# PROBIC/mSWEEP

Hardware: AMD Instinct MI355X
Metric: EM iters/sec + reads×groups cells/sec, 10M reads × 5k groups (higher is better)
Workload: dtype f64

## Files before the change

include/msweep_core.h:

```cpp
#ifndef MSWEEP_CORE_H
#define MSWEEP_CORE_H

#include <stddef.h>
#include <stdint.h>

#ifdef __cplusplus
extern "C" {
#endif

typedef struct msw_core *msw_handle;

enum { MSW_ALGO_RCG = 0, MSW_ALGO_EM = 1 };
enum { MSW_PREC_DOUBLE = 0, MSW_PREC_FLOAT = 1 };

int msw_core_create(int device, msw_handle *out);
void msw_core_destroy(msw_handle h);
const char *msw_last_error(msw_handle h);
const char *msw_core_version(void);


int msw_core_set_dense_logl(msw_handle h, const double *L, size_t n_groups, size_t n_ecs,
                            size_t ld);

int msw_core_set_csr(msw_handle h, const uint64_t *rowptr, const uint32_t *grp,
// ... 15 lines not shown
  int32_t record_bytes;
  int32_t index_records;
  int32_t groups_in_lds;
  int32_t table_in_lds;
  int32_t passB_mode;
  uint32_t slot_entries;
  uint32_t slot_entries_in_lds;
  uint32_t n_slices, n_long_ecs;
  uint64_t rows;
  uint64_t rows_from_memory;
  uint32_t slices_by_lanes[7];
  uint32_t max_rows;
  int32_t bank_scheduled;
  int32_t passB_reg_cells;
  uint64_t rows_over_8;
} msw_layout_info;
int msw_core_layout_info(msw_handle h, msw_layout_info *out);
int msw_core_set_pack_schedule(msw_handle h, int enabled);

enum { MSW_OPT_CHECK_EVERY = 0, MSW_OPT_INIT_BOUND = 1, MSW_OPT_EM_PRIOR = 2, MSW_OPT_EM_STOP = 3 };
int msw_core_set_option(msw_handle h, int option, double value);
int msw_core_get_option(msw_handle h, int option, double *value);

int msw_core_solve(msw_handle h, const double *logc, const double *alpha0, double tol,
                   size_t max_iters, int algo, int prec, double *theta_out,
                   size_t *iters_out, double *bound_out);

int msw_core_prepare(msw_handle h, const double *logc, const double *alpha0);
int msw_core_run(msw_handle h, double tol, size_t max_iters, int algo, int prec,
                 double *theta_out, size_t *iters_out, double *bound_out);

int msw_core_gamma(msw_handle h, double *gamma_out, size_t ld);
// ... 127 lines not shown
```

msweep_amd/core.py:

```python
import ctypes as C
import os

import numpy as np

_HERE = os.path.dirname(os.path.abspath(__file__))
LIB_PATH = os.environ.get("MSWEEP_CORE_LIB") or os.path.join(_HERE, "libmsweep_core.so")

ALGO_RCG, ALGO_EM = 0, 1
PREC_DOUBLE, PREC_FLOAT = 0, 1
TEXT_PROBS, TEXT_LOGL, TEXT_BITSEQ = 0, 1, 2
OPT_CHECK_EVERY, OPT_INIT_BOUND, OPT_EM_PRIOR, OPT_EM_STOP = 0, 1, 2, 3
_OPTS = {"check_every": OPT_CHECK_EVERY, "init_bound": OPT_INIT_BOUND, "em_prior": OPT_EM_PRIOR, "em_stop": OPT_EM_STOP}

EXPORTS = [
    "msw_core_create", "msw_core_destroy", "msw_last_error", "msw_core_version",
    "msw_core_set_dense_logl", "msw_core_set_csr", "msw_core_build_likelihood",
    "msw_core_get_dense_logl", "msw_core_layout_hash", "msw_core_shape", "msw_alignment_read",
    "msw_alignment_shape", "msw_alignment_export", "msw_alignment_view", "msw_alignment_destroy", "msw_alignment_last_error",
    "msw_alignment_read_device", "msw_core_build_likelihood_aln", "msw_core_trim", "msw_alignment_on_device", "msw_core_solve", "msw_core_prepare", "msw_core_run",
    "msw_core_gamma",
    "msw_core_trace", "msw_core_set_trace_theta", "msw_core_bootstrap",
    "msw_core_resample_counts", "msw_core_set_profiling", "msw_core_last_timing",
    "msw_core_set_fixed_iters", "msw_core_hbm_stream_rates", "msw_comm_unique_id", "msw_comm_create_rccl", "msw_comm_create_local",
    "msw_comm_destroy", "msw_core_set_comm", "msw_comm_last_error", "msw_core_bootstrap_dist",
    "msw_comm_size", "msw_comm_rccl_count", "msw_comm_allgather", "msw_comm_allreduce", "msw_comm_create_shm", "msw_core_continue", "msw_core_gamma_block",
    "msw_core_last_bootstrap_timing", "msw_core_layout_info", "msw_core_guarded_visits", "msw_core_set_pack_schedule",
    "msw_core_set_option", "msw_core_get_option", "msw_core_bin_reads", "msw_core_bin_reads_aln",
    "msw_core_text_block", "msw_core_format_g6", "msw_core_last_text_timing",
    "msw_core_gzip_begin", "msw_core_text_block_gzip", "msw_core_gzip_append", "msw_core_gzip_end", "msw_core_last_gzip_timing",
    "msw_core_inflate_gzip", "msw_alignment_last_inflate",
]

INFLATE_REASONS = ("none", "forced", "header", "probe mismatch", "chunk status", "crc", "trailing bytes", "memory", "long span")


class MswError(RuntimeError):
    """Non-zero return from the C ABI (mirrors the std::runtime_error the C++ shim throws)."""


class InflateInfo(C.Structure):
    _fields_ = [("payload_bytes", C.c_uint64), ("text_bytes", C.c_uint64), ("chunk_bytes", C.c_uint32), ("n_chunks", C.c_uint32),
                ("n_starts", C.c_uint32), ("on_device", C.c_int32), ("fallback_reason", C.c_int32), ("n_members", C.c_uint32),
                ("kernel_ms", C.c_double),
                ("upload_ms", C.c_double), ("probe_ms", C.c_double), ("window_ms", C.c_double), ("chain_ms", C.c_double),
                ("write_ms", C.c_double), ("crc_ms", C.c_double)]
# ... 5 lines not shown


class Timing(C.Structure):
    _fields_ = [("solve_ms", C.c_double), ("passA_ms", C.c_double), ("passB_ms", C.c_double),
                ("passA_launches", C.c_uint64), ("passB_launches", C.c_uint64), ("iters", C.c_uint64),
                ("bytes_passA", C.c_uint64), ("bytes_passB", C.c_uint64), ("collective_ms", C.c_double),
                ("collectives", C.c_uint64), ("em_float_kernels", C.c_uint64)]


class LayoutInfo(C.Structure):
    _fields_ = [("record_bytes", C.c_int32), ("index_records", C.c_int32), ("groups_in_lds", C.c_int32),
                ("table_in_lds", C.c_int32), ("passB_mode", C.c_int32), ("slot_entries", C.c_uint32),
                ("slot_entries_in_lds", C.c_uint32), ("n_slices", C.c_uint32), ("n_long_ecs", C.c_uint32),
                ("rows", C.c_uint64), ("rows_from_memory", C.c_uint64), ("slices_by_lanes", C.c_uint32 * 7),
                ("max_rows", C.c_uint32), ("bank_scheduled", C.c_int32), ("passB_reg_cells", C.c_int32),
                ("rows_over_8", C.c_uint64)]


class BootstrapTiming(C.Structure):
    _fields_ = [("table_ms", C.c_double), ("solve_ms", C.c_double), ("gather_ms", C.c_double),
                ("replicates", C.c_uint64), ("iterations", C.c_uint64), ("table_reused", C.c_uint64)]


_lib = None


def source_hash():
    import hashlib
    csrc = os.path.join(_HERE, "csrc")
    h = hashlib.sha256()
    files = sorted(os.path.join(csrc, f) for f in os.listdir(csrc) if f.endswith((".hip", ".hpp", ".inc", ".h")))
# ... 66 lines not shown
    L.msw_comm_size.argtypes = [vp, C.POINTER(C.c_int), C.POINTER(C.c_int)]
    L.msw_comm_rccl_count.argtypes = [vp, C.POINTER(C.c_int)]
    L.msw_comm_allgather.argtypes = [vp, vp, sz, vp]
    L.msw_comm_allreduce.argtypes = [vp, vp, sz, vp, sz, C.c_int, C.POINTER(dp)]
    L.msw_comm_create_shm.argtypes = [C.c_char_p, C.c_int, C.c_int, C.c_int, C.POINTER(vp)]
    L.msw_core_set_profiling.argtypes = [vp, C.c_int]
    L.msw_core_set_fixed_iters.argtypes = [vp, C.c_int]
    L.msw_core_set_pack_schedule.argtypes = [vp, C.c_int]
    L.msw_core_set_option.argtypes = [vp, C.c_int, C.c_double]
    L.msw_core_get_option.argtypes = [vp, C.c_int, C.POINTER(C.c_double)]
    L.msw_core_hbm_stream_rates.argtypes = [vp, C.c_size_t, C.c_int, C.POINTER(C.c_double), C.POINTER(C.c_double)]
    L.msw_core_last_timing.argtypes = [vp, C.POINTER(Timing)]
    L.msw_core_last_bootstrap_timing.argtypes = [vp, C.POINTER(BootstrapTiming)]
    L.msw_core_guarded_visits.argtypes = [vp, C.POINTER(C.c_uint64)]
    L.msw_core_layout_info.argtypes = [vp, C.POINTER(LayoutInfo)]
    L.msw_comm_unique_id.argtypes = [vp]
    L.msw_comm_create_rccl.argtypes = [vp, C.c_int, C.c_int, C.c_int, C.POINTER(vp)]
    L.msw_comm_create_local.argtypes = [C.c_int, C.POINTER(vp)]
    L.msw_comm_destroy.argtypes = [vp]
    L.msw_comm_destroy.restype = None
    L.msw_core_set_comm.argtypes = [vp, vp]
    L.msw_comm_last_error.restype = C.c_char_p
    L.msw_alignment_read.argtypes = [C.POINTER(C.c_char_p), sz, sz, C.c_int, C.POINTER(vp)]
    L.msw_alignment_shape.argtypes = [vp, C.POINTER(sz), C.POINTER(sz), C.POINTER(sz), C.POINTER(sz)]
    L.msw_alignment_view.argtypes = [vp] + [C.POINTER(vp)] * 5
    L.msw_alignment_export.argtypes = [vp, vp, vp, vp, vp, vp]
    L.msw_alignment_destroy.argtypes = [vp]
    L.msw_core_trim.argtypes = [vp]
    L.msw_alignment_on_device.argtypes = [vp]
    L.msw_alignment_read_device.argtypes = [vp, C.POINTER(C.c_char_p), sz, sz, C.c_int, C.POINTER(vp)]
# ... 190 lines not shown
        self._check(self._L.msw_core_build_likelihood_aln(
            self._h, aln._h, _ptr(target_group), len(target_group), _ptr(group_sizes), G, q, e, zero_inflation,
            int(min_hits), C.byref(n_out), _ptr(mask), _ptr(logc)))
        return n_out.value, mask.astype(bool), logc

    def shape(self):
        g, e, n = C.c_size_t(), C.c_size_t(), C.c_size_t()
        self._check(self._L.msw_core_shape(self._h, C.byref(g), C.byref(e), C.byref(n)))
        return g.value, e.value, n.value

    def layout_info(self):
        t = LayoutInfo()
        self._check(self._L.msw_core_layout_info(self._h, C.byref(t)))
        return {k: (list(getattr(t, k)) if k == "slices_by_lanes" else getattr(t, k)) for k, _ in LayoutInfo._fields_}

    def layout_hash(self):
        out = C.c_uint64(0)
        self._check(self._L.msw_core_layout_hash(self._h, C.byref(out)))
        return int(out.value)

    def get_dense_logl(self):
        G, E, _ = self.shape()
        out = np.empty((G, E))
        self._check(self._L.msw_core_get_dense_logl(self._h, _ptr(out), E))
        return out

    def solve(self, logc, alpha0, tol=1e-6, max_iters=5000, algo=ALGO_RCG, prec=PREC_DOUBLE):
        G, E, _ = self.shape()
        logc = None if logc is None else _arr(logc, np.float64)
        alpha0 = _arr(alpha0, np.float64)
# ... 323 lines not shown
```

msweep_amd/csrc/common.hpp:

```cpp
#pragma once
#include <hip/hip_runtime.h>

#include <cstdint>
#include <cstdio>
#include <stdexcept>
#include <string>
#include <vector>

namespace msw {

constexpr int kWave = 64;
#ifndef MSW_PASS_THREADS_A
#define MSW_PASS_THREADS_A 1024
#endif
#ifndef MSW_PASS_THREADS_B
#define MSW_PASS_THREADS_B 768
#endif
#ifndef MSW_PASS_THREADS_B8
#define MSW_PASS_THREADS_B8 1024
#endif
constexpr int kPassThreads = MSW_PASS_THREADS_A;
constexpr int kPassThreadsB = MSW_PASS_THREADS_B;
constexpr int kPassThreadsB8 = MSW_PASS_THREADS_B8;
constexpr int kMaxTrace = 4096;
// ... 59 lines not shown
  int32_t em_prior = 0;
  int32_t em_stop = 0;
};

#ifdef MSW_STAMPS
__device__ unsigned long long g_stamps[64 * 40];
#define MSW_STAMP(it, K, p) (g_stamps[((it) & 63) * 40 + (K) * 8 + (p)] = __builtin_amdgcn_s_memrealtime())
#define MSW_STAMP_MAX(it, K, p) atomicMax(&g_stamps[((it) & 63) * 40 + (K) * 8 + (p)], (unsigned long long)__builtin_amdgcn_s_memrealtime())
#else
#define MSW_STAMP(it, K, p) ((void)0)
#define MSW_STAMP_MAX(it, K, p) ((void)0)
#endif

struct TabDev {
  double2 *A, *B;
};

struct Scalars {
  double a, os_a, step_a;
  double oldnorm, newnorm, beta;
  double bound, oldbound, bound_const;
  double tol, csum;
  double M, U, p0, kappa;
  double logzi;
  double fx_scale, fx_inv, fx_tscale, fx_tinv, xb, tmax, tmin;
  double tref;
  int32_t didreset, reset_pending, done, iter;
  int32_t have_eval, eval_pad;
  int32_t max_iters, fixed_iters, trace_theta, flavor;
  int32_t check_every, em_prior, em_stop, opt_pad;
  int32_t tab_ver, fx_shift;
// ... 4 lines not shown
```

msweep_amd/csrc/host_em.inc:

```
namespace {

void run_em(const Resident &L, Solver &s, size_t max_iters, int prec) {
  const int G = (int)L.G, n_lut = L.n_tab_inline();
  TraceDev tr{s.tr_bound.p, s.tr_newnorm.p, s.tr_beta.p, s.tr_theta.p, s.tr_reset.p};
  hipLaunchKernelGGL(k_em_init, dim3(1), dim3(1024), 0, s.stream, s.sc.p, G, n_lut, s.u.p, L.lut_area.p,
                     s.e.p, s.tabs());
  launch_tables(L, s);
  const bool f32 = prec == MSW_PREC_FLOAT && em_f32_layout_ok(L, s);
  struct Flag {
    Solver &s;
    ~Flag() { s.em_f32 = false; }
  } flag{s};
  s.em_f32 = f32;
  s.timing.em_float_kernels = f32 ? 1 : 0;
  if (f32) {
    s.e32.alloc((size_t)G + kSentinels);
    s.tab32.alloc(std::max<uint32_t>(L.n_area, 1));
    hipLaunchKernelGGL(k_em_f32_prep, dim3(1), dim3(1024), 0, s.stream, s.sc.p, G, (int)L.n_area, L.lut_area.p, s.e.p,
                       s.e32.p, s.tab32.p);
  }
  size_t enq = 0;
  while (enq < max_iters) {
    const size_t batch = std::min<size_t>(kIterBatch, max_iters - enq);
    for (size_t b = 0; b < batch; ++b) {
      launch_passB(L, s);
      hipLaunchKernelGGL(k_em_fin, dim3(1), dim3(1024), 0, s.stream, s.sc.p, G, n_lut, fin_npartS(L, s), fin_partS(L, s),
                         s.Nc.p, s.alpha0.p, s.u.p, s.logth.p, L.lut_area.p, s.e.p, s.tabs(), tr,
                         f32 ? s.e32.p : (float *)nullptr);
    }
    MSW_HIP(hipGetLastError());
    enq += batch;
    poll(s);
    if (s.sc_host->done) break;
  }
}

}
```

msweep_amd/csrc/host_likelihood.inc:

```
namespace {

void sell_from_device(msw_core *h, const uint32_t *d_rowptr, const uint32_t *d_grp, const uint32_t *d_idx,
                      const double *cell_val = nullptr);
bool compress_dense(msw_core *h, const double *Lm, size_t ld, const double *stage, size_t G, size_t E, bool force);

void reset_likelihood(msw_core *h) {
  Resident &L = h->lik;
  static_cast<LikShape &>(L) = LikShape{};
  h->solver.have_solution = false;
  h->solver.prepared = false;
  h->iperm.release();
  L.long_row = multilane() ? kLongRow : kLongRowOneLane;
  if (const char *lr = getenv("MSWEEP_LONG_ROW"))
    L.long_row = (uint32_t)std::min(std::max(atoi(lr), 16), (int)L.long_row);
}

constexpr uint8_t kRGroup[64] = {0, 0, 0, 0, 1, 1, 1, 1, 1, 1, 1, 1, 0, 0, 0, 0, 1, 1, 1, 1, 0, 0,
                                 0, 0, 0, 0, 0, 0, 1, 1, 1, 1, 2, 2, 2, 2, 3, 3, 3, 3, 3, 3, 3, 3,
                                 2, 2, 2, 2, 3, 3, 3, 3, 2, 2, 2, 2, 2, 2, 2, 2, 3, 3, 3, 3};

constexpr uint8_t kRPos[64] = {0, 1, 2,  3,  0,  1,  2,  3,  4,  5,  6,  7,  4,  5,  6,  7,  8,  9,  10, 11, 8, 9,
                               10, 11, 12, 13, 14, 15, 12, 13, 14, 15, 0,  1,  2,  3,  0,  1,  2,  3,  4,  5, 6, 7,
                               4,  5,  6,  7,  8,  9,  10, 11, 8,  9,  10, 11, 12, 13, 14, 15, 12, 13, 14, 15};

struct SlotPlan {
  std::vector<uint32_t> canon, hot_rank;
  uint32_t rep_base = 0, H = 0, sentinel_slot = 0;
};
SlotPlan plan_slot_area(msw_core *h, const std::vector<uint64_t> &freq) {
  Resident &L = h->lik;
  const uint32_t n_lut = L.n_lut;
  SlotPlan sp;
  std::vector<uint32_t> used;
  for (uint32_t i = 0; i < n_lut; ++i) if (freq[i]) used.push_back(i);
  if (used.empty()) used.push_back(0);
  std::vector<uint32_t> by_freq(used);
  std::stable_sort(by_freq.begin(), by_freq.end(), [&](uint32_t a, uint32_t b) { return freq[a] > freq[b]; });
  sp.canon.assign(std::max<uint32_t>(n_lut, 1), 0);
  sp.hot_rank.assign(std::max<uint32_t>(n_lut, 1), UINT32_MAX);
  sp.sentinel_slot = used[0];
  for (uint32_t tryH : {64u, 32u, 16u, 8u, 0u}) {
    if (tryH > used.size()) continue;
    sp.H = tryH;
    sp.rep_base = sp.H ? (uint32_t)((used.size() + 15) & ~(size_t)15) : (uint32_t)used.size();
    L.n_area = sp.rep_base + 8 * sp.H;
    choose_layout(L);
    if (L.tlds && L.glds && !L.wide()) break;
  }
  bool hybrid = false;
  if (!L.tlds) {
    sp.H = 0;
    sp.rep_base = (uint32_t)used.size();
    L.n_area = (uint32_t)used.size();
    choose_layout(L);
    hybrid = choose_hybrid_layout(L, h->no_hybrid);
    if (hybrid) sp.sentinel_slot = by_freq[0];
  }
  const std::vector<uint32_t> &order = hybrid ? by_freq : used;
  std::vector<uint32_t> area_slot(L.n_area, used[0]);
  for (uint32_t e = 0; e < order.size(); ++e) area_slot[e] = order[e], sp.canon[order[e]] = e;
  for (uint32_t j = 0; j < sp.H; ++j) {
    sp.hot_rank[by_freq[j]] = j;
    for (uint32_t c = 0; c < 8; ++c) area_slot[sp.rep_base + (j >> 1) * 16 + 2 * c + (j & 1)] = by_freq[j];
  }
  L.area_slot.upload(area_slot.data(), area_slot.size(), h->stream);
  L.lut_area.alloc(L.n_area);
  hipLaunchKernelGGL(k_gather_f64, dim3((L.n_area + 255) / 256), dim3(256), 0, h->stream, L.lut.p, L.area_slot.p,
                     L.n_area, L.lut_area.p);
  L.trange.alloc(2);
  hipLaunchKernelGGL(k_minmax, dim3(1), dim3(1024), 0, h->stream, L.lut_area.p, (uint64_t)L.n_area, 0, L.trange.p);
  MSW_HIP(hipGetLastError());
  MSW_HIP(hipStreamSynchronize(h->stream));
  return sp;
}

void finish_sell(msw_core *h) {
  Resident &L = h->lik;
  const uint32_t wg_for_slices = (L.nslices + (kPassThreads / 64) - 1) / (kPassThreads / 64);
  L.nblk = (int)std::max<uint32_t>(1, std::min<uint32_t>(std::max(wg_for_slices, L.n_long), (uint32_t)h->n_cu));
// ... 25 lines not shown
  const uint32_t E = L.E, G = L.G, n_lut = L.n_lut;
  const uint64_t nnz_all = rowptr[E];
  std::vector<uint64_t> freq(std::max<uint32_t>(n_lut, 1), 0);
  for (uint64_t k = 0; k < nnz_all; ++k) ++freq[cell_idx[k]];
  const SlotPlan sp = plan_slot_area(h, freq);
  const std::vector<uint32_t> &canon = sp.canon, &hot_rank = sp.hot_rank;
  const uint32_t rep_base = sp.rep_base;
  const std::vector<uint32_t> used = {sp.sentinel_slot};
  const bool wide = L.wide(), hybrid = L.hybrid();
  const int rw = wide ? 2 : 1;
  const RecDec dec = L.dec;
  const uint32_t n_hot = L.n_tab_lds;
  auto entry_of = [&](int lane, uint32_t idx) -> uint32_t {
    const uint32_t j = hot_rank[idx];
    if (lane < 0 || j == UINT32_MAX) return canon[idx];
    return rep_base + (j >> 1) * 16 + 2 * (kRPos[lane] >> 1) + (j & 1);
  };
  auto put_entry = [&](std::vector<uint32_t> &dst, size_t slot, uint32_t g, uint32_t entry, bool hot = false) {
    if (wide) {
      const uint2 r = Rec<kEncWide>::make(g, entry, dec);
      dst[2 * slot] = r.x;
      dst[2 * slot + 1] = r.y;
    } else if (hybrid) {
      dst[slot] = hot ? Rec<kEncIndex>::make_h(g, entry, dec) : Rec<kEncIndex>::make(g, entry, dec);
    } else {
      dst[slot] = Rec<kEncNarrow>::make(g, entry, dec);
    }
  };
  auto put = [&](std::vector<uint32_t> &dst, size_t slot, uint32_t g, uint32_t idx, int lane, bool hot = false) {
    put_entry(dst, slot, g, entry_of(lane, idx), hot);
  };
// ... 444 lines not shown
```

msweep_amd/csrc/host_pack.inc:

```
namespace {

uint64_t device_scan_u32(msw_core *h, uint32_t *d, uint64_t n, DevBuf<uint32_t> &tot, DevBuf<uint64_t> &gt);

void choose_value_layout(Resident &L) {
  L.enc = kEncValue;
  L.tlds = false;
  L.n_area = 0;
  L.n_tab_lds = 0;
  L.dec.shift = 0;
  L.dec.mask = 0;
  L.dec.bhi = L.dec.bhiA = 0;
  const char *force = getenv("MSWEEP_FORCE_LDS");
  const bool want_glds = !(force && strlen(force) == 2 && force[0] == '0');
  L.glds = want_glds && pass_lds_bytes(1, 0, L.G, true, false) <= kLdsMax && passB_mode(L, true, 0, false) >= 0;
  L.gmodeB = passB_mode(L, L.glds, 0, false);
  if (L.gmodeB < 0) throw Fail("internal: no LDS configuration fits");
  if (8ull * ((uint64_t)L.G + kSentinels) >= (1ull << 31)) throw Fail("likelihood too large: group offsets exceed the record field");
}

void sell_from_device(msw_core *h, const uint32_t *d_rowptr, const uint32_t *d_grp, const uint32_t *d_idx,
                      const double *cell_val ) {
  Resident &L = h->lik;
  const uint32_t E = L.E, n_lut = L.n_lut;
  const uint64_t nnz = L.nnz;
// ... 81 lines not shown
      sell_from_device(h, d_rowptr, d_grp, d_idx, cell_val);
    } catch (...) {
      h->no_hybrid = false;
      throw;
    }
    h->no_hybrid = false;
    return;
  }
  const size_t nslots = (size_t)n_rows * 64;
  if (L.hybrid()) L.slice_hot.alloc(std::max<uint32_t>(nslices, 1));
  L.rec.alloc(rec_words(L.enc, nslots + 64) + 2);
  L.rec_long.alloc(rec_words(L.enc, (size_t)n_long_cells + 64) + 2);
  MSW_HIP(hipMemsetAsync(L.rec.p + rec_words(L.enc, nslots), 0, (rec_words(L.enc, 64) + 2) * sizeof(uint32_t), st));
  MSW_HIP(hipMemsetAsync(L.rec_long.p, 0, (rec_words(L.enc, (size_t)n_long_cells + 64) + 2) * sizeof(uint32_t), st));
  tm.mark("  pack: geometry + alloc");
  const PackEnc pe{d_canon.p, d_hot.p, sp.rep_base, L.G, sp.sentinel_slot, L.dec, L.n_tab_lds, L.slice_hot.p,
                   cell_val, L.logzi};
  if (n_long) {
    auto k = L.enc == kEncValue ? k_pack_long<kEncValue>
                                 : (L.wide() ? k_pack_long<kEncWide> : (L.hybrid() ? k_pack_long<kEncIndex> : k_pack_long<kEncNarrow>));
    hipLaunchKernelGGL(k, dim3(std::min<uint32_t>(n_long, (uint32_t)h->n_cu * 32)), dim3(64), 0, st, d_rowptr, d_grp, d_idx,
                       L.perm.p, L.long_ptr.p, n_long, pe, L.rec_long.p);
  }
  if (nslices) {
    auto k = L.enc == kEncValue ? k_pack_slices<kEncValue>
                                 : (L.wide() ? k_pack_slices<kEncWide> : (L.hybrid() ? k_pack_slices<kEncIndex> : k_pack_slices<kEncNarrow>));
    hipLaunchKernelGGL(k, dim3(std::min<uint32_t>(nslices, (uint32_t)h->n_cu * 64)), dim3(64), 0, st, d_rowptr, d_grp,
                       d_idx, L.perm.p, L.slice_off.p, n_long, n_sell, nslices, L.cls, pe, h->pack_schedule ? 1 : 0, L.rec.p);
  }
  MSW_HIP(hipGetLastError());
  tm.mark("  pack: records");
// ... 39 lines not shown
```

msweep_amd/csrc/msweep_core.hip:

```cpp
#include "../../include/msweep_core.h"

#include <algorithm>
#include <array>
#include <cmath>
#include <chrono>
#include <cstring>
#include <limits>
#include <memory>
#include <string>
#include <thread>
#include <unordered_map>
#include <vector>

#include <zlib.h>

#include <rocprim/device/device_radix_sort.hpp>
#include <rocprim/device/device_scan.hpp>
#include <rocprim/iterator/counting_iterator.hpp>
#include <rocprim/iterator/transform_iterator.hpp>

#include "kernels.hpp"
#include "pack_kernels.hpp"
#include "compress_kernels.hpp"
#include "comm.hpp"
// ... 18 lines not shown
constexpr size_t kLdsMax = 160 * 1024;
constexpr int kIterBatch = 16;
}


struct LikShape {
  int flavor = -1;
  uint32_t G = 0, E = 0, n_lut = 0, nslices = 0, n_long = 0;
  uint64_t nnz = 0, nslots = 0;
  int enc = kEncNarrow;
  bool glds = true, tlds = true;
  int gmodeB = 1;
  RecDec dec = {};
  uint32_t n_area = 0;
  uint32_t n_tab_lds = 0;
  SliceClasses cls = {};
  bool packed_scheduled = false;
  uint32_t long_row = kLongRow;
  uint64_t rows_over8 = 0;
  bool passB_rc8 = false;
  double logzi = 0.0;
  int nblk = 0;
  int nblk_dense = 0;
  int nreg = 0;
  bool have_logc_res = false;
};

struct Resident : LikShape {
  DevBuf<uint32_t> rec, slice_off, long_ptr, rec_long, perm;
  DevBuf<uint8_t> slice_hot;
// ... 16 lines not shown

struct Solver {
  hipStream_t stream = nullptr;
  int n_cu = 256;
  msw_comm *const *commp;
  bool *collective;
  explicit Solver(msw_comm *const *c = nullptr, bool *coll = nullptr) : commp(c), collective(coll) {}
  msw_comm *comm() const { return commp ? *commp : nullptr; }
  SolveOpts opts;
  bool profiling = false, fixed_iters = false;
  size_t trace_theta = 0;

  DevBuf<double> cvec, logc_d, alpha0, u, os_u, step_u, w, e, N, Nc, Acc;
  DevBuf<uint8_t> c8, c8s;
  DevBuf<double2> ew, tabA, tabB;
  TabDev tabs() const { return TabDev{tabA.p, tabB.p}; }
  DevBuf<int> tab_built;
  DevBuf<double> partA, partS, partAcc, partC, partR, totS;
  size_t lds_attr[3][80] = {};
  DevBuf<double> commA, commB;
  DevBuf<uint32_t> guard_list, guard_bits;
  DevBuf<unsigned long long> guard_tail;
  DevBuf<int> guard_err;
  DevBuf<unsigned long long> guard_visits;
  DevBuf<Scalars> sc;
  Scalars *sc_host = nullptr;
  DevBuf<double> tr_bound, tr_newnorm, tr_beta, tr_theta;
  DevBuf<int32_t> tr_reset;
  bool have_solution = false;
  bool prepared = false;
  int last_algo = MSW_ALGO_RCG;
// ... 589 lines not shown
                       s.alpha0.p, s.Nc.p, s.N.p, s.w.p, s.ew.p, s.partR.p, s.totS.p);
    return;
  }
  hipLaunchKernelGGL(k_redfin, dim3((L.G + kRedfinGroups - 1) / kRedfinGroups), dim3(kRedfinThreads), 0, s.stream,
                     s.sc.p, (int)L.G, partials ? nb : 0, fxrows, fxrows ? s.guard_tail.p : nullptr, 1, nb,
                     s.partAcc.p, s.Acc.p, s.partS.p, s.e.p,
                     s.u.p, s.alpha0.p, s.Nc.p, s.N.p, s.w.p, s.ew.p, s.partR.p, s.totS.p);
}

const double *fin_partS(const Resident &L, Solver &s) { return s.comm() ? s.commB.p + 3 * (size_t)L.G : s.partS.p; }
int fin_npartS(const Resident &L, Solver &s) { return s.comm() ? 1 : L.npart_rows(); }

void launch_tables(const Resident &L, Solver &s) {
  if (L.flavor != 0 || L.n_area <= (uint32_t)kTabInline) return;
  const unsigned nb = std::min<unsigned>((L.n_area + 255) / 256, (unsigned)s.n_cu * 8);
  hipLaunchKernelGGL(k_tables, dim3(nb), dim3(256), 0, s.stream, s.sc.p, (int)L.n_area, L.lut_area.p, s.tabs(),
                     s.tab_built.p);
}

void launch_finstep(const Resident &L, Solver &s, int mode) {
  TraceDev tr{s.tr_bound.p, s.tr_newnorm.p, s.tr_beta.p, s.tr_theta.p, s.tr_reset.p};
  const double *pA = s.partA.p;
  int npA = L.flavor == 0 ? L.nblk : L.nblk_dense;
  if (s.comm()) {
    pA = s.commA.p;
    npA = 1;
  }
  hipLaunchKernelGGL(k_finstep, dim3(1), dim3(1024), 0, s.stream, s.sc.p, mode, (int)L.G, L.n_tab_inline(), npA, pA,
                     (int)((L.G + kRedfinGroups - 1) / kRedfinGroups), s.totS.p, s.partR.p, s.Nc.p, s.w.p, s.u.p,
                     s.os_u.p, s.step_u.p, L.lut_area.p, s.e.p, s.tabs(), tr);
  launch_tables(L, s);
}

void poll(Solver &s) {
  MSW_HIP(hipMemcpyAsync(s.sc_host, s.sc.p, sizeof(Scalars), hipMemcpyDeviceToHost, s.stream));
  MSW_HIP(hipStreamSynchronize(s.stream));
  if (s.comm()) s.comm()->check();
}

constexpr int kCvecBlocks = 512;
void prepare_inputs(const Resident &L, Solver &s, const double *logc_host, const uint32_t *counts_dev,
                    const double *alpha0_host) {
  if (L.flavor < 0) throw Fail("no likelihood resident: call msw_core_set_csr / set_dense_logl first");
  const uint32_t E = L.E, G = L.G;
  if (counts_dev) {
// ... 39 lines not shown
    cpart = s.commA.p;
    ncpart = 1;
  }
  hipLaunchKernelGGL(k_init_state, dim3(1), dim3(1024), 0, s.stream, s.sc.p, (int)G, ncpart,
                     cpart, s.alpha0.p, s.u.p, s.os_u.p, s.step_u.p, tol, (int)max_iters,
                     s.fixed_iters ? 1 : 0, (int)s.trace_theta, L.flavor, L.logzi, s.opts, s.tab_built.p,
                     L.trange.p);
  MSW_HIP(hipGetLastError());
}

void run_rcg(const Resident &L, Solver &s, size_t max_iters, size_t iters_start = 0) {
  const int G = (int)L.G, n_lut = L.n_tab_inline();
  if (iters_start > 0 && s.comm()) s.comm()->rendezvous();
  if (iters_start == 0) {
    hipLaunchKernelGGL(k_prepB, dim3(1), dim3(1024), 0, s.stream, s.sc.p, G, n_lut, s.u.p, L.lut_area.p,
                       s.e.p, s.tabs());
    launch_tables(L, s);
    launch_passB(L, s);
    s.timing.passB_launches--;
    if (s.profiling && s.evB_used) s.evB_used--;
  }
  const int nbA = L.flavor == 0 ? L.nblk : L.nblk_dense;
  size_t iters_done = iters_start;
  for (;;) {
    const size_t missing = std::max<size_t>(1, max_iters - std::min(max_iters, iters_done));
    const size_t batch = s.fixed_iters ? std::min<size_t>(256, missing) : std::min<size_t>(kIterBatch, missing);
    for (size_t b = 0; b < batch; ++b) {
      launch_passA(L, s);
      if (s.comm()) {
        std::pair<hipEvent_t, hipEvent_t> *evc = nullptr;
        if (s.profiling) {
// ... 311 lines not shown
    const Resident &L = h->lik;
    if (L.flavor != 0) throw Fail("msw_core_layout_info: no CSR-of-ECs likelihood resident");
    msw_layout_info li = {};
    li.record_bytes = L.enc == kEncValue ? 12 : (L.wide() ? 8 : 4);
    li.index_records = L.hybrid() ? 1 : 0;
    li.groups_in_lds = L.glds ? 1 : 0;
    li.table_in_lds = L.tlds ? 1 : 0;
    li.passB_mode = L.gmodeB;
    li.slot_entries = L.n_area;
    li.slot_entries_in_lds = L.n_tab_lds;
    li.n_slices = L.nslices;
    li.n_long_ecs = L.n_long;
    li.bank_scheduled = L.packed_scheduled ? 1 : 0;
    li.passB_reg_cells = L.passB_rc8 ? 8 : kRegCells;
    li.rows_over_8 = L.rows_over8;
    std::vector<uint32_t> off((size_t)L.nslices + 1);
    MSW_HIP(hipMemcpy(off.data(), L.slice_off.p, off.size() * sizeof(uint32_t), hipMemcpyDeviceToHost));
    li.rows = off[L.nslices];
    for (int c = 0; c < kSliceClasses; ++c) li.slices_by_lanes[c] = L.cls.s0[c + 1] - L.cls.s0[c];
    for (uint32_t s2 = 0; s2 < L.nslices; ++s2) li.max_rows = std::max(li.max_rows, off[s2 + 1] - off[s2]);
    if (L.hybrid()) {
      std::vector<uint8_t> hot(std::max<uint32_t>(L.nslices, 1));
      MSW_HIP(hipMemcpy(hot.data(), L.slice_hot.p, hot.size(), hipMemcpyDeviceToHost));
      for (uint32_t s2 = 0; s2 < L.nslices; ++s2) li.rows_from_memory += (off[s2 + 1] - off[s2]) - hot[s2];
    } else if (!L.tlds && L.enc != kEncValue) {
      li.rows_from_memory = li.rows;
    }
    *out = li;
  });
}

int msw_core_layout_hash(msw_handle h, uint64_t *hash_out) {
  return guarded(h, [&] {
    if (!hash_out) throw Fail("null out");
    *hash_out = layout_hash(h->lik);
  });
}

int msw_core_get_dense_logl(msw_handle h, double *L_out, size_t ld) {
  return guarded(h, [&] { materialise_impl(h, L_out, ld, false, 0, h->lik.E); });
}

int msw_core_gamma(msw_handle h, double *gamma_out, size_t ld) {
// ... 441 lines not shown
```

msweep_amd/csrc/pack_kernels.hpp:

```cpp
#pragma once
#include "common.hpp"
#include "sell.hpp"

namespace msw {

__device__ __constant__ uint8_t kRGroupDev[64] = {0, 0, 0, 0, 1, 1, 1, 1, 1, 1, 1, 1, 0, 0, 0, 0, 1, 1, 1, 1, 0, 0,
                                                  0, 0, 0, 0, 0, 0, 1, 1, 1, 1, 2, 2, 2, 2, 3, 3, 3, 3, 3, 3, 3, 3,
                                                  2, 2, 2, 2, 3, 3, 3, 3, 2, 2, 2, 2, 2, 2, 2, 2, 3, 3, 3, 3};
__device__ __constant__ uint8_t kRPosDev[64] = {0,  1,  2,  3,  0,  1,  2,  3,  4,  5,  6,  7,  4,  5,  6,  7,
                                                8,  9,  10, 11, 8,  9,  10, 11, 12, 13, 14, 15, 12, 13, 14, 15,
                                                0,  1,  2,  3,  0,  1,  2,  3,  4,  5,  6,  7,  4,  5,  6,  7,
                                                8,  9,  10, 11, 8,  9,  10, 11, 12, 13, 14, 15, 12, 13, 14, 15};

__host__ __device__ inline uint32_t cold_class(uint32_t n_cold) {
  return n_cold == 0 ? 0u : (n_cold <= 2 ? 1u : (n_cold <= (uint32_t)kColdRows ? 2u : 3u));
}
constexpr uint32_t kPackKeyBits = 13;
__global__ __launch_bounds__(256) void k_pack_keys(const uint32_t *rowptr, uint32_t E, uint32_t long_row, int multilane,
                                                  const uint32_t *idx, const uint32_t *canon, uint32_t n_hot,
                                                  uint32_t *key, uint32_t *val, uint32_t *counts) {
  uint32_t mine[1 + kSliceClasses] = {};
  for (uint32_t j = blockIdx.x * blockDim.x + threadIdx.x; j < E; j += gridDim.x * blockDim.x) {
    const uint32_t b = rowptr[j], len = rowptr[j + 1] - b;
    const bool lg = len > long_row;
// ... 54 lines not shown
    __syncthreads();
    for (uint32_t i = threadIdx.x; i < n_lut; i += blockDim.x)
      if (hist[i]) atomicAdd(&freq[i], (unsigned long long)hist[i]);
  }
}

__global__ __launch_bounds__(256) void k_gather_f64(const double *src, const uint32_t *at, uint32_t n, double *dst) {
  const uint32_t i = blockIdx.x * blockDim.x + threadIdx.x;
  if (i < n) dst[i] = src[at[i]];
}

struct PackEnc {
  const uint32_t *canon;
  const uint32_t *hot_rank;
  uint32_t rep_base, n_groups, sentinel_slot;
  RecDec dec;
  uint32_t n_hot;
  uint8_t *slice_hot;
  const double *cell_val;
  double tnull;
};
constexpr uint32_t kPackPad = UINT32_MAX;
__device__ __forceinline__ uint32_t pack_entry(const PackEnc &pe, int lane, uint32_t idx) {
  if (pe.cell_val) return idx;
  const uint32_t j = pe.hot_rank[idx];
  if (lane < 0 || j == UINT32_MAX) return pe.canon[idx];
  return pe.rep_base + (j >> 1) * 16 + 2 * (kRPosDev[lane] >> 1) + (j & 1);
}
template <int ENC>
__device__ __forceinline__ void pack_put(uint32_t *dst, size_t slot, const PackEnc &pe, uint32_t g, uint32_t entry,
                                         bool hot = false) {
  if constexpr (ENC == kEncValue) {
    Rec<ENC>::store(dst, slot, ValRec{8u * g, entry == kPackPad ? pe.tnull : pe.cell_val[entry]});
  } else {
    if (entry == kPackPad) entry = pe.canon[pe.sentinel_slot];
    if constexpr (ENC == kEncIndex) dst[slot] = hot ? Rec<ENC>::make_h(g, entry, pe.dec) : Rec<ENC>::make(g, entry, pe.dec);
    else reinterpret_cast<typename Rec<ENC>::T *>(dst)[slot] = Rec<ENC>::make(g, entry, pe.dec);
  }
}

constexpr uint32_t kLongResidues = 32;
__host__ __device__ inline uint32_t long_cell_pos(const uint32_t *b, uint32_t r, uint32_t j) {
// ... 196 lines not shown
```

msweep_amd/csrc/state_kernels.hpp:

```cpp
#pragma once
#include "device_util.hpp"

namespace msw {

struct TraceDev {
  double *bound, *newnorm, *beta, *theta;
  int32_t *didreset;
};

__device__ inline void prepB_block(Scalars *sc, double a, int G, int n_lut, const double *u,
                                   const double *lut, double *e, TabDev X, double *sh) {
  const int tid = threadIdx.x, nt = blockDim.x;
  double m = -INFINITY;
  for (int g = tid; g < G; g += nt) m = fmax(m, u[g]);
  const double M = block_max(m, sh);
  double su = 0.0;
  for (int g = tid; g < G; g += nt) {
    const double eg = flush_denormal(exp(u[g] - M));
    e[g] = eg;
    su += eg;
  }
  const double U = block_sum(su, sh);
  const double logzi = sc->logzi, oma = 1.0 - a;
  const double tref = tref_of(a, sc->tmax, sc->tmin);
  const double p0 = exp(a * (logzi - tref));
  const double xtop = 1.0;
  for (int i = tid; i < n_lut; i += nt) {
    const double T = lut[i], x = exp(a * (T - tref));
    X.A[i] = make_double2(x, oma * (T - logzi));
    X.B[i] = make_double2(x - p0, x * T - p0 * logzi);
  }
  if (tid == 0) {
    sc->M = M;
    sc->U = U;
    sc->p0 = p0;
    sc->tref = tref;
    sc->xb = fmax(xtop, p0);
    sc->fx_shift = fx_shift_of(fmax(xtop, p0), p0);
    sc->tab_ver = sc->tab_ver + 1;
  }
}

constexpr int kTabInline = 16384;
__global__ __launch_bounds__(256) void k_tables(const Scalars *sc, int n_tab, const double *lut, TabDev X,
                                               int *built) {
// ... 43 lines not shown
  __shared__ double sh[32];
  if (sc->done) return;
  if (sc->flavor != 0) return;
  const double a = sc->a;
  __syncthreads();
  prepB_block(sc, a, G, n_lut, u, lut, e, X, sh);
}

constexpr int kStepRegs = 6;
__global__ __launch_bounds__(1024) void k_finstep(Scalars *sc, int mode, int G, int n_lut, int n_partA,
                                                 const double *partA, int npartR, const double *totS,
                                                 const double *partR, const double *Nc, const double *w, double *u,
                                                 double *os_u, double *step_u, const double *lut, double *e, TabDev X,
                                                 TraceDev tr) {
  __shared__ double sh[16 * (kRedfinParts + 1)];
  const int tid = threadIdx.x, nt = blockDim.x;
  const bool inreg = G <= kStepRegs * nt;
  double q[kRedfinParts + 1] = {0.0, 0.0, 0.0, 0.0, 0.0, 0.0};
  for (int b = tid; b < npartR; b += nt)
    for (int i = 0; i < kRedfinParts; ++i) q[i] += partR[kRedfinParts * b + i];
  for (int i = tid; i < n_partA; i += nt) q[kRedfinParts] += partA[i];
  const double s_clogZ = totS[0], s_rH = totS[1];
  double wv[kStepRegs], sv[kStepRegs], uv[kStepRegs];
  if (inreg) {
#pragma unroll
    for (int k = 0; k < kStepRegs; ++k) {
      const int g = tid + k * nt;
      if (g < G) {
        wv[k] = w[g];
        sv[k] = step_u[g];
        uv[k] = u[g];
      }
    }
  }
  const double lt = tid < n_lut ? lut[tid] : 0.0;
  if (tid == 0) MSW_STAMP(sc->iter, 1, 0);
  const Scalars s0 = *sc;
  if (s0.done) return;
  block_sum_fixed<kRedfinParts + 1, 16>(q, sh);
  if (tid == 0) MSW_STAMP(s0.iter, 1, 2);
  const double lg = q[0], mu = q[1], S0 = q[2], S1 = q[3], pnsum = q[5];
  const int flavor = s0.flavor;
  const double logzi = s0.logzi;
  double a = s0.a, os_a = s0.os_a, kappa = s0.kappa, bound = s0.bound;
  int didreset = s0.didreset, it = s0.iter, done = 0;
  bool old_is_step = false;

  if (s0.have_eval == 2) {
    if (flavor == 0) kappa += S1 / S0;
  } else if (s0.have_eval == 1) {
// ... 122 lines not shown
        osu *= beta;
        su += osu;
      }
      uv[k] += su;
      os_u[g] = osu;
      step_u[g] = su;
      u[g] = uv[k];
      m = fmax(m, uv[k]);
    }
  }
  double p0 = 0.0, tref = 0.0;
  if (flavor == 0) {
    const double oma = 1.0 - a_new;
    tref = tref_of(a_new, s0.tmax, s0.tmin);
    p0 = exp(a_new * (logzi - tref));
    for (int i = tid; i < n_lut; i += nt) {
      const double T = i == tid ? lt : lut[i], x = exp(a_new * (T - tref));
      X.A[i] = make_double2(x, oma * (T - logzi));
      X.B[i] = make_double2(x - p0, x * T - p0 * logzi);
    }
  }
  double M = 0.0, U = 0.0;
  if (flavor == 0) {
    M = block_max_fixed<16>(m, sh);
    double su = 0.0;
#pragma unroll
    for (int k = 0; k < kStepRegs; ++k) {
      const int g = tid + k * nt;
      if (g < G) {
        const double eg = flush_denormal(exp(uv[k] - M));
        e[g] = eg;
        su += eg;
      }
    }
    U = block_sum_fixed1<16>(su, sh);
  }
  if (tid == 0) MSW_STAMP(s0.iter, 1, 6);
  if (tid == 0) {
    sc->a = a_new;
// ... 351 lines not shown
```

Before: 241700 billion.

## Generalize hot-slot replication and compute replicated table entries once

Moves the slot-replica index math into a shared header and adds an optional 16-replica layout that allows up to 192 hot slots, selected by environment variable. The default stays at 8 paired replicas with 64 hot slots. Table-building kernels now compute each hot entry once into shared memory and then spread it to its replica positions, avoiding redundant exp evaluations. This adds a shared-memory staging buffer, an extra spread pass, and a debug export of the slot tables.

Measured after the change: 238500 billion. 1.3% lower.

```diff
diff --git a/include/msweep_core.h b/include/msweep_core.h
--- a/include/msweep_core.h
+++ b/include/msweep_core.h
@@ -53,8 +53,12 @@
   int32_t bank_scheduled;
   int32_t passB_reg_cells;
   uint64_t rows_over_8;
+  uint32_t slot_replicated;
+  uint32_t slot_replicas;
+  uint32_t slot_replica_base;
 } msw_layout_info;
 int msw_core_layout_info(msw_handle h, msw_layout_info *out);
+int msw_core_slot_tables(msw_handle h, uint32_t *area_slot_out, double *tabA_out, double *tabB_out, size_t n);
 int msw_core_set_pack_schedule(msw_handle h, int enabled);
 
 enum { MSW_OPT_CHECK_EVERY = 0, MSW_OPT_INIT_BOUND = 1, MSW_OPT_EM_PRIOR = 2, MSW_OPT_EM_STOP = 3 };
diff --git a/msweep_amd/core.py b/msweep_amd/core.py
--- a/msweep_amd/core.py
+++ b/msweep_amd/core.py
@@ -28,7 +28,7 @@
     "msw_core_set_option", "msw_core_get_option", "msw_core_bin_reads", "msw_core_bin_reads_aln",
     "msw_core_text_block", "msw_core_format_g6", "msw_core_last_text_timing",
     "msw_core_gzip_begin", "msw_core_text_block_gzip", "msw_core_gzip_append", "msw_core_gzip_end", "msw_core_last_gzip_timing",
-    "msw_core_inflate_gzip", "msw_alignment_last_inflate",
+    "msw_core_inflate_gzip", "msw_alignment_last_inflate", "msw_core_slot_tables",
 ]
 
 INFLATE_REASONS = ("none", "forced", "header", "probe mismatch", "chunk status", "crc", "trailing bytes", "memory", "long span")
@@ -64,7 +64,8 @@
                 ("slot_entries_in_lds", C.c_uint32), ("n_slices", C.c_uint32), ("n_long_ecs", C.c_uint32),
                 ("rows", C.c_uint64), ("rows_from_memory", C.c_uint64), ("slices_by_lanes", C.c_uint32 * 7),
                 ("max_rows", C.c_uint32), ("bank_scheduled", C.c_int32), ("passB_reg_cells", C.c_int32),
-                ("rows_over_8", C.c_uint64)]
+                ("rows_over_8", C.c_uint64), ("slot_replicated", C.c_uint32), ("slot_replicas", C.c_uint32),
+                ("slot_replica_base", C.c_uint32)]
 
 
 class BootstrapTiming(C.Structure):
@@ -161,6 +162,8 @@
     L.msw_core_last_bootstrap_timing.argtypes = [vp, C.POINTER(BootstrapTiming)]
     L.msw_core_guarded_visits.argtypes = [vp, C.POINTER(C.c_uint64)]
     L.msw_core_layout_info.argtypes = [vp, C.POINTER(LayoutInfo)]
+    if hasattr(L, "msw_core_slot_tables"):
+        L.msw_core_slot_tables.argtypes = [vp, vp, vp, vp, sz]
     L.msw_comm_unique_id.argtypes = [vp]
     L.msw_comm_create_rccl.argtypes = [vp, C.c_int, C.c_int, C.c_int, C.POINTER(vp)]
     L.msw_comm_create_local.argtypes = [C.c_int, C.POINTER(vp)]
@@ -381,6 +384,12 @@
         self._check(self._L.msw_core_layout_info(self._h, C.byref(t)))
         return {k: (list(getattr(t, k)) if k == "slices_by_lanes" else getattr(t, k)) for k, _ in LayoutInfo._fields_}
 
+    def slot_tables(self):
+        n = self.layout_info()["slot_entries"]
+        slot, A, B = np.zeros(n, np.uint32), np.zeros((n, 2)), np.zeros((n, 2))
+        self._check(self._L.msw_core_slot_tables(self._h, _ptr(slot), _ptr(A), _ptr(B), n))
+        return slot, A, B
+
     def layout_hash(self):
         out = C.c_uint64(0)
         self._check(self._L.msw_core_layout_hash(self._h, C.byref(out)))
diff --git a/msweep_amd/csrc/common.hpp b/msweep_amd/csrc/common.hpp
--- a/msweep_amd/csrc/common.hpp
+++ b/msweep_amd/csrc/common.hpp
@@ -6,6 +6,8 @@
 #include <stdexcept>
 #include <string>
 #include <vector>
+
+#include "slot_entry.hpp"
 
 namespace msw {
 
@@ -97,7 +99,34 @@
 
 struct TabDev {
   double2 *A, *B;
+  uint32_t rep_base, n_hot, nrep;
 };
+struct TabHot {
+  double2 a[kSlotHotMax], b[kSlotHotMax];
+};
+__device__ __forceinline__ int tab_items(const TabDev &X, int n_tab) {
+  return n_tab && X.n_hot ? (int)(X.rep_base + X.n_hot) : n_tab;
+}
+__device__ __forceinline__ int tab_item_src(const TabDev &X, int i) {
+  return !X.n_hot || i < (int)X.rep_base ? i : (int)slot_replica_copy(X.nrep, X.rep_base, (uint32_t)i - X.rep_base, 0);
+}
+__device__ __forceinline__ void tab_item_store(const TabDev &X, TabHot &hot, int i, double2 a, double2 b) {
+  if (!X.n_hot || i < (int)X.rep_base) {
+    X.A[i] = a;
+    X.B[i] = b;
+  } else {
+    hot.a[i - (int)X.rep_base] = a;
+    hot.b[i - (int)X.rep_base] = b;
+  }
+}
+__device__ __forceinline__ void tab_spread(const TabDev &X, const TabHot &hot, int n_tab) {
+  if (!X.n_hot) return;
+  for (int e = (int)X.rep_base + (int)threadIdx.x; e < n_tab; e += (int)blockDim.x) {
+    const uint32_t j = slot_replica_rank(X.nrep, X.rep_base, (uint32_t)e);
+    X.A[e] = hot.a[j];
+    X.B[e] = hot.b[j];
+  }
+}
 
 struct Scalars {
   double a, os_a, step_a;
diff --git a/msweep_amd/csrc/host_em.inc b/msweep_amd/csrc/host_em.inc
--- a/msweep_amd/csrc/host_em.inc
+++ b/msweep_amd/csrc/host_em.inc
@@ -4,7 +4,7 @@
   const int G = (int)L.G, n_lut = L.n_tab_inline();
   TraceDev tr{s.tr_bound.p, s.tr_newnorm.p, s.tr_beta.p, s.tr_theta.p, s.tr_reset.p};
   hipLaunchKernelGGL(k_em_init, dim3(1), dim3(1024), 0, s.stream, s.sc.p, G, n_lut, s.u.p, L.lut_area.p,
-                     s.e.p, s.tabs());
+                     s.e.p, s.tabs(L));
   launch_tables(L, s);
   const bool f32 = prec == MSW_PREC_FLOAT && em_f32_layout_ok(L, s);
   struct Flag {
@@ -25,7 +25,7 @@
     for (size_t b = 0; b < batch; ++b) {
       launch_passB(L, s);
       hipLaunchKernelGGL(k_em_fin, dim3(1), dim3(1024), 0, s.stream, s.sc.p, G, n_lut, fin_npartS(L, s), fin_partS(L, s),
-                         s.Nc.p, s.alpha0.p, s.u.p, s.logth.p, L.lut_area.p, s.e.p, s.tabs(), tr,
+                         s.Nc.p, s.alpha0.p, s.u.p, s.logth.p, L.lut_area.p, s.e.p, s.tabs(L), tr,
                          f32 ? s.e32.p : (float *)nullptr);
     }
     MSW_HIP(hipGetLastError());
diff --git a/msweep_amd/csrc/host_likelihood.inc b/msweep_amd/csrc/host_likelihood.inc
--- a/msweep_amd/csrc/host_likelihood.inc
+++ b/msweep_amd/csrc/host_likelihood.inc
@@ -15,17 +15,10 @@
     L.long_row = (uint32_t)std::min(std::max(atoi(lr), 16), (int)L.long_row);
 }
 
-constexpr uint8_t kRGroup[64] = {0, 0, 0, 0, 1, 1, 1, 1, 1, 1, 1, 1, 0, 0, 0, 0, 1, 1, 1, 1, 0, 0,
-                                 0, 0, 0, 0, 0, 0, 1, 1, 1, 1, 2, 2, 2, 2, 3, 3, 3, 3, 3, 3, 3, 3,
-                                 2, 2, 2, 2, 3, 3, 3, 3, 2, 2, 2, 2, 2, 2, 2, 2, 3, 3, 3, 3};
-
-constexpr uint8_t kRPos[64] = {0, 1, 2,  3,  0,  1,  2,  3,  4,  5,  6,  7,  4,  5,  6,  7,  8,  9,  10, 11, 8, 9,
-                               10, 11, 12, 13, 14, 15, 12, 13, 14, 15, 0,  1,  2,  3,  0,  1,  2,  3,  4,  5, 6, 7,
-                               4,  5,  6,  7,  8,  9,  10, 11, 8,  9,  10, 11, 12, 13, 14, 15, 12, 13, 14, 15};
-
 struct SlotPlan {
   std::vector<uint32_t> canon, hot_rank;
   uint32_t rep_base = 0, H = 0, sentinel_slot = 0;
+  uint32_t nrep = kSlotReplicasDefault;
 };
 SlotPlan plan_slot_area(msw_core *h, const std::vector<uint64_t> &freq) {
   Resident &L = h->lik;
@@ -39,11 +32,14 @@
   sp.canon.assign(std::max<uint32_t>(n_lut, 1), 0);
   sp.hot_rank.assign(std::max<uint32_t>(n_lut, 1), UINT32_MAX);
   sp.sentinel_slot = used[0];
-  for (uint32_t tryH : {64u, 32u, 16u, 8u, 0u}) {
-    if (tryH > used.size()) continue;
+  if (const char *e = getenv("MSWEEP_SLOT_REPLICAS")) sp.nrep = atoi(e) == 16 ? kSlotReplicas : (atoi(e) == 8 ? kSlotReplicasPaired : sp.nrep);
+  uint32_t maxH = sp.nrep == kSlotReplicas ? kSlotHotMax : kSlotHotMaxPaired;
+  if (const char *e = getenv("MSWEEP_SLOT_HOT")) maxH = std::min<uint32_t>(maxH, (uint32_t)std::max(atoi(e), 0));
+  for (uint32_t tryH : {192u, 128u, 64u, 32u, 16u, 8u, 0u}) {
+    if (tryH > used.size() || tryH > maxH) continue;
     sp.H = tryH;
     sp.rep_base = sp.H ? (uint32_t)((used.size() + 15) & ~(size_t)15) : (uint32_t)used.size();
-    L.n_area = sp.rep_base + 8 * sp.H;
+    L.n_area = slot_area_entries(sp.nrep, sp.rep_base, sp.H);
     choose_layout(L);
     if (L.tlds && L.glds && !L.wide()) break;
   }
@@ -61,8 +57,11 @@
   for (uint32_t e = 0; e < order.size(); ++e) area_slot[e] = order[e], sp.canon[order[e]] = e;
   for (uint32_t j = 0; j < sp.H; ++j) {
     sp.hot_rank[by_freq[j]] = j;
-    for (uint32_t c = 0; c < 8; ++c) area_slot[sp.rep_base + (j >> 1) * 16 + 2 * c + (j & 1)] = by_freq[j];
-  }
+    for (uint32_t c = 0; c < sp.nrep; ++c) area_slot[slot_replica_copy(sp.nrep, sp.rep_base, j, c)] = by_freq[j];
+  }
+  L.rep_base = sp.H ? sp.rep_base : L.n_area;
+  L.n_rep_hot = sp.H;
+  L.nrep = sp.nrep;
   L.area_slot.upload(area_slot.data(), area_slot.size(), h->stream);
   L.lut_area.alloc(L.n_area);
   hipLaunchKernelGGL(k_gather_f64, dim3((L.n_area + 255) / 256), dim3(256), 0, h->stream, L.lut.p, L.area_slot.p,
@@ -118,7 +117,7 @@
   auto entry_of = [&](int lane, uint32_t idx) -> uint32_t {
     const uint32_t j = hot_rank[idx];
     if (lane < 0 || j == UINT32_MAX) return canon[idx];
-    return rep_base + (j >> 1) * 16 + 2 * (kRPos[lane] >> 1) + (j & 1);
+    return slot_replica_entry(sp.nrep, rep_base, j, kRPos[lane]);
   };
   auto put_entry = [&](std::vector<uint32_t> &dst, size_t slot, uint32_t g, uint32_t entry, bool hot = false) {
     if (wide) {
diff --git a/msweep_amd/csrc/host_pack.inc b/msweep_amd/csrc/host_pack.inc
--- a/msweep_amd/csrc/host_pack.inc
+++ b/msweep_amd/csrc/host_pack.inc
@@ -119,7 +119,7 @@
   MSW_HIP(hipMemsetAsync(L.rec.p + rec_words(L.enc, nslots), 0, (rec_words(L.enc, 64) + 2) * sizeof(uint32_t), st));
   MSW_HIP(hipMemsetAsync(L.rec_long.p, 0, (rec_words(L.enc, (size_t)n_long_cells + 64) + 2) * sizeof(uint32_t), st));
   tm.mark("  pack: geometry + alloc");
-  const PackEnc pe{d_canon.p, d_hot.p, sp.rep_base, L.G, sp.sentinel_slot, L.dec, L.n_tab_lds, L.slice_hot.p,
+  const PackEnc pe{d_canon.p, d_hot.p, sp.rep_base, L.G, sp.sentinel_slot, sp.nrep, L.dec, L.n_tab_lds, L.slice_hot.p,
                    cell_val, L.logzi};
   if (n_long) {
     auto k = L.enc == kEncValue ? k_pack_long<kEncValue>
diff --git a/msweep_amd/csrc/msweep_core.hip b/msweep_amd/csrc/msweep_core.hip
--- a/msweep_amd/csrc/msweep_core.hip
+++ b/msweep_amd/csrc/msweep_core.hip
@@ -56,6 +56,7 @@
   RecDec dec = {};
   uint32_t n_area = 0;
   uint32_t n_tab_lds = 0;
+  uint32_t rep_base = 0, n_rep_hot = 0, nrep = kSlotReplicasDefault;
   SliceClasses cls = {};
   bool packed_scheduled = false;
   uint32_t long_row = kLongRow;
@@ -102,7 +103,7 @@
   DevBuf<double> cvec, logc_d, alpha0, u, os_u, step_u, w, e, N, Nc, Acc;
   DevBuf<uint8_t> c8, c8s;
   DevBuf<double2> ew, tabA, tabB;
-  TabDev tabs() const { return TabDev{tabA.p, tabB.p}; }
+  TabDev tabs(const Resident &L) const { return TabDev{tabA.p, tabB.p, L.rep_base, L.n_rep_hot, L.nrep}; }
   DevBuf<int> tab_built;
   DevBuf<double> partA, partS, partAcc, partC, partR, totS;
   size_t lds_attr[3][80] = {};
@@ -722,7 +723,7 @@
 void launch_tables(const Resident &L, Solver &s) {
   if (L.flavor != 0 || L.n_area <= (uint32_t)kTabInline) return;
   const unsigned nb = std::min<unsigned>((L.n_area + 255) / 256, (unsigned)s.n_cu * 8);
-  hipLaunchKernelGGL(k_tables, dim3(nb), dim3(256), 0, s.stream, s.sc.p, (int)L.n_area, L.lut_area.p, s.tabs(),
+  hipLaunchKernelGGL(k_tables, dim3(nb), dim3(256), 0, s.stream, s.sc.p, (int)L.n_area, L.lut_area.p, s.tabs(L),
                      s.tab_built.p);
 }
 
@@ -736,7 +737,7 @@
   }
   hipLaunchKernelGGL(k_finstep, dim3(1), dim3(1024), 0, s.stream, s.sc.p, mode, (int)L.G, L.n_tab_inline(), npA, pA,
                      (int)((L.G + kRedfinGroups - 1) / kRedfinGroups), s.totS.p, s.partR.p, s.Nc.p, s.w.p, s.u.p,
-                     s.os_u.p, s.step_u.p, L.lut_area.p, s.e.p, s.tabs(), tr);
+                     s.os_u.p, s.step_u.p, L.lut_area.p, s.e.p, s.tabs(L), tr);
   launch_tables(L, s);
 }
 
@@ -806,7 +807,7 @@
   if (iters_start > 0 && s.comm()) s.comm()->rendezvous();
   if (iters_start == 0) {
     hipLaunchKernelGGL(k_prepB, dim3(1), dim3(1024), 0, s.stream, s.sc.p, G, n_lut, s.u.p, L.lut_area.p,
-                       s.e.p, s.tabs());
+                       s.e.p, s.tabs(L));
     launch_tables(L, s);
     launch_passB(L, s);
     s.timing.passB_launches--;
@@ -1148,6 +1149,9 @@
     li.bank_scheduled = L.packed_scheduled ? 1 : 0;
     li.passB_reg_cells = L.passB_rc8 ? 8 : kRegCells;
     li.rows_over_8 = L.rows_over8;
+    li.slot_replicated = L.n_rep_hot;
+    li.slot_replicas = L.n_rep_hot ? L.nrep : 0;
+    li.slot_replica_base = L.rep_base;
     std::vector<uint32_t> off((size_t)L.nslices + 1);
     MSW_HIP(hipMemcpy(off.data(), L.slice_off.p, off.size() * sizeof(uint32_t), hipMemcpyDeviceToHost));
     li.rows = off[L.nslices];
@@ -1161,6 +1165,18 @@
       li.rows_from_memory = li.rows;
     }
     *out = li;
+  });
+}
+
+int msw_core_slot_tables(msw_handle h, uint32_t *area_slot_out, double *tabA_out, double *tabB_out, size_t n) {
+  return guarded(h, [&] {
+    const Resident &L = h->lik;
+    if (L.flavor != 0 || L.enc == kEncValue) throw Fail("msw_core_slot_tables: no likelihood with a slot area resident");
+    if (n != L.n_area || !area_slot_out || !tabA_out || !tabB_out) throw Fail("msw_core_slot_tables: n must be slot_entries, the outputs non-null");
+    MSW_HIP(hipStreamSynchronize(h->stream));
+    MSW_HIP(hipMemcpy(area_slot_out, L.area_slot.p, n * sizeof(uint32_t), hipMemcpyDeviceToHost));
+    MSW_HIP(hipMemcpy(tabA_out, h->solver.tabA.p, n * sizeof(double2), hipMemcpyDeviceToHost));
+    MSW_HIP(hipMemcpy(tabB_out, h->solver.tabB.p, n * sizeof(double2), hipMemcpyDeviceToHost));
   });
 }
 
diff --git a/msweep_amd/csrc/pack_kernels.hpp b/msweep_amd/csrc/pack_kernels.hpp
--- a/msweep_amd/csrc/pack_kernels.hpp
+++ b/msweep_amd/csrc/pack_kernels.hpp
@@ -92,6 +92,7 @@
   const uint32_t *canon;
   const uint32_t *hot_rank;
   uint32_t rep_base, n_groups, sentinel_slot;
+  uint32_t nrep;
   RecDec dec;
   uint32_t n_hot;
   uint8_t *slice_hot;
@@ -103,7 +104,7 @@
   if (pe.cell_val) return idx;
   const uint32_t j = pe.hot_rank[idx];
   if (lane < 0 || j == UINT32_MAX) return pe.canon[idx];
-  return pe.rep_base + (j >> 1) * 16 + 2 * (kRPosDev[lane] >> 1) + (j & 1);
+  return slot_replica_entry(pe.nrep, pe.rep_base, j, kRPosDev[lane]);
 }
 template <int ENC>
 __device__ __forceinline__ void pack_put(uint32_t *dst, size_t slot, const PackEnc &pe, uint32_t g, uint32_t entry,
diff --git a/msweep_amd/csrc/slot_entry.hpp b/msweep_amd/csrc/slot_entry.hpp
--- /dev/null
+++ b/msweep_amd/csrc/slot_entry.hpp
@@ -0,0 +1,36 @@
+#pragma once
+#include <cstdint>
+
+#if defined(__HIPCC__) || defined(__CUDACC__)
+#define MSW_SLOT_HD __host__ __device__
+#else
+#define MSW_SLOT_HD
+#endif
+
+namespace msw {
+
+constexpr uint8_t kRGroup[64] = {0, 0, 0, 0, 1, 1, 1, 1, 1, 1, 1, 1, 0, 0, 0, 0, 1, 1, 1, 1, 0, 0,
+                                 0, 0, 0, 0, 0, 0, 1, 1, 1, 1, 2, 2, 2, 2, 3, 3, 3, 3, 3, 3, 3, 3,
+                                 2, 2, 2, 2, 3, 3, 3, 3, 2, 2, 2, 2, 2, 2, 2, 2, 3, 3, 3, 3};
+
+constexpr uint8_t kRPos[64] = {0, 1, 2,  3,  0,  1,  2,  3,  4,  5,  6,  7,  4,  5,  6,  7,  8,  9,  10, 11, 8, 9,
+                               10, 11, 12, 13, 14, 15, 12, 13, 14, 15, 0,  1,  2,  3,  0,  1,  2,  3,  4,  5, 6, 7,
+                               4,  5,  6,  7,  8,  9,  10, 11, 8,  9,  10, 11, 12, 13, 14, 15, 12, 13, 14, 15};
+
+constexpr uint32_t kSlotReplicas = 16, kSlotReplicasPaired = 8;
+constexpr uint32_t kSlotReplicasDefault = kSlotReplicasPaired;
+constexpr uint32_t kSlotHotMax = 192, kSlotHotMaxPaired = 64;
+
+MSW_SLOT_HD inline uint32_t slot_replica_entry(uint32_t nrep, uint32_t rep_base, uint32_t j, uint32_t pos) {
+  return nrep == kSlotReplicas ? rep_base + 16u * j + pos : rep_base + (j >> 1) * 16u + 2u * (pos >> 1) + (j & 1u);
+}
+MSW_SLOT_HD inline uint32_t slot_replica_copy(uint32_t nrep, uint32_t rep_base, uint32_t j, uint32_t c) {
+  return slot_replica_entry(nrep, rep_base, j, nrep == kSlotReplicas ? c : 2u * c);
+}
+MSW_SLOT_HD inline uint32_t slot_replica_rank(uint32_t nrep, uint32_t rep_base, uint32_t e) {
+  const uint32_t d = e - rep_base;
+  return nrep == kSlotReplicas ? d >> 4 : ((d >> 4) << 1) | (d & 1u);
+}
+MSW_SLOT_HD inline uint32_t slot_area_entries(uint32_t nrep, uint32_t rep_base, uint32_t H) { return rep_base + nrep * H; }
+
+}
diff --git a/msweep_amd/csrc/state_kernels.hpp b/msweep_amd/csrc/state_kernels.hpp
--- a/msweep_amd/csrc/state_kernels.hpp
+++ b/msweep_amd/csrc/state_kernels.hpp
@@ -25,10 +25,20 @@
   const double tref = tref_of(a, sc->tmax, sc->tmin);
   const double p0 = exp(a * (logzi - tref));
   const double xtop = 1.0;
-  for (int i = tid; i < n_lut; i += nt) {
-    const double T = lut[i], x = exp(a * (T - tref));
-    X.A[i] = make_double2(x, oma * (T - logzi));
-    X.B[i] = make_double2(x - p0, x * T - p0 * logzi);
+  if (!X.n_hot) {
+    for (int i = tid; i < n_lut; i += nt) {
+      const double T = lut[i], x = exp(a * (T - tref));
+      X.A[i] = make_double2(x, oma * (T - logzi));
+      X.B[i] = make_double2(x - p0, x * T - p0 * logzi);
+    }
+  } else {
+    __shared__ TabHot hot;
+    for (int i = tid, n = tab_items(X, n_lut); i < n; i += nt) {
+      const double T = lut[tab_item_src(X, i)], x = exp(a * (T - tref));
+      tab_item_store(X, hot, i, make_double2(x, oma * (T - logzi)), make_double2(x - p0, x * T - p0 * logzi));
+    }
+    __syncthreads();
+    tab_spread(X, hot, n_lut);
   }
   if (tid == 0) {
     sc->M = M;
@@ -102,6 +112,7 @@
                                                  double *os_u, double *step_u, const double *lut, double *e, TabDev X,
                                                  TraceDev tr) {
   __shared__ double sh[16 * (kRedfinParts + 1)];
+  __shared__ TabHot hot;
   const int tid = threadIdx.x, nt = blockDim.x;
   const bool inreg = G <= kStepRegs * nt;
   double q[kRedfinParts + 1] = {0.0, 0.0, 0.0, 0.0, 0.0, 0.0};
@@ -121,7 +132,8 @@
       }
     }
   }
-  const double lt = tid < n_lut ? lut[tid] : 0.0;
+  const int n_tab = tab_items(X, n_lut);
+  const double lt = tid < n_tab ? lut[tab_item_src(X, tid)] : 0.0;
   if (tid == 0) MSW_STAMP(sc->iter, 1, 0);
   const Scalars s0 = *sc;
   if (s0.done) return;
@@ -274,15 +286,23 @@
     const double oma = 1.0 - a_new;
     tref = tref_of(a_new, s0.tmax, s0.tmin);
     p0 = exp(a_new * (logzi - tref));
-    for (int i = tid; i < n_lut; i += nt) {
-      const double T = i == tid ? lt : lut[i], x = exp(a_new * (T - tref));
-      X.A[i] = make_double2(x, oma * (T - logzi));
-      X.B[i] = make_double2(x - p0, x * T - p0 * logzi);
+    if (!X.n_hot) {
+      for (int i = tid; i < n_lut; i += nt) {
+        const double T = i == tid ? lt : lut[i], x = exp(a_new * (T - tref));
+        X.A[i] = make_double2(x, oma * (T - logzi));
+        X.B[i] = make_double2(x - p0, x * T - p0 * logzi);
+      }
+    } else {
+      for (int i = tid; i < n_tab; i += nt) {
+        const double T = i == tid ? lt : lut[tab_item_src(X, i)], x = exp(a_new * (T - tref));
+        tab_item_store(X, hot, i, make_double2(x, oma * (T - logzi)), make_double2(x - p0, x * T - p0 * logzi));
+      }
     }
   }
   double M = 0.0, U = 0.0;
   if (flavor == 0) {
     M = block_max_fixed<16>(m, sh);
+    tab_spread(X, hot, n_lut);
     double su = 0.0;
 #pragma unroll
     for (int k = 0; k < kStepRegs; ++k) {
```
